# HorizonRobotics/GeoFlowSlam

Hardware: AMD Instinct MI355X
Metric: front-end frames/sec (ORB+match+GICP) on 640x480 RGBD (higher is better)
Workload: dtype u8/int32 (ORB, match) + f64 (GICP); 1 GPU; BASELINE.json configs[1]: 640x480 RGBD frame pair, ORB extract (1000 feats, 8 levels) + BF Hamming match + GMS filter + GICP on ~19k-pt clouds (stride-4 depth grid); batch_pairs_per_gpu=512, lanes_per_gpu=4, passes=K passes per lane chain, joined once, distinct_scenes_per_gpu=512, scene_seeds=1000..1511 (rank 0), global_batch_pairs=512, parallelism=frames sharded x1, no collective

## Files before the change

### geoflowslam_amd/csrc/match.hip

```cpp
#include "gfs_common.hpp"

namespace {

constexpr int kQPerBlock = 64;
constexpr int kTile = 256;

__global__ __launch_bounds__(256) void k_bf_hamming(const uint8_t* __restrict__ query, const int* __restrict__ nq_arr,
                                                    const uint8_t* __restrict__ train, const int* __restrict__ nt_arr,
                                                    int stride_rows, int* __restrict__ out_idx,
                                                    int* __restrict__ out_dist) {
  __shared__ uint4 tile[kTile * 2];
  __shared__ unsigned int part[4][kQPerBlock];
  const int b = blockIdx.y;
  const int nq = nq_arr[b], nt = nt_arr[b];
  const int q0 = blockIdx.x * kQPerBlock;
  if (q0 >= nq) return;
  const int lane = threadIdx.x & 63, wave = threadIdx.x >> 6;
  const int q = q0 + lane;
  const uint8_t* qb = query + (size_t)b * stride_rows * 32;
  const uint8_t* tb = train + (size_t)b * stride_rows * 32;

  unsigned long long qa[4] = {0, 0, 0, 0};
  if (q < nq) {
    const uint4* qp = reinterpret_cast<const uint4*>(qb + (size_t)q * 32);
    uint4 lo = qp[0], hi = qp[1];
    qa[0] = (unsigned long long)lo.x | ((unsigned long long)lo.y << 32);
    qa[1] = (unsigned long long)lo.z | ((unsigned long long)lo.w << 32);
    qa[2] = (unsigned long long)hi.x | ((unsigned long long)hi.y << 32);
    qa[3] = (unsigned long long)hi.z | ((unsigned long long)hi.w << 32);
  }
  int best = 0x7fffffff, best_j = -1;
  for (int t0 = 0; t0 < nt; t0 += kTile) {
    __syncthreads();
    const uint4* src = reinterpret_cast<const uint4*>(tb + (size_t)t0 * 32);
    const int rows = min(kTile, nt - t0);
    for (int i = threadIdx.x; i < rows * 2; i += 256) tile[i] = src[i];
    __syncthreads();
    const int r0 = wave * 64, r1 = min(r0 + 64, rows);
    for (int r = r0; r < r1; ++r) {
      uint4 lo = tile[2 * r], hi = tile[2 * r + 1];
      unsigned long long t0w = (unsigned long long)lo.x | ((unsigned long long)lo.y << 32);
      unsigned long long t1w = (unsigned long long)lo.z | ((unsigned long long)lo.w << 32);
      unsigned long long t2w = (unsigned long long)hi.x | ((unsigned long long)hi.y << 32);
      unsigned long long t3w = (unsigned long long)hi.z | ((unsigned long long)hi.w << 32);
      int d = __popcll(qa[0] ^ t0w) + __popcll(qa[1] ^ t1w) + __popcll(qa[2] ^ t2w) + __popcll(qa[3] ^ t3w);
      if (d < best) {
        best = d;
        best_j = t0 + r;
      }
    }
  }
  part[wave][lane] = best_j < 0 ? 0xffffffffu : ((unsigned int)best << 20) | (unsigned int)best_j;
  __syncthreads();
  if (wave == 0 && q < nq) {
    unsigned int k = min(min(part[0][lane], part[1][lane]), min(part[2][lane], part[3][lane]));
    int* oi = out_idx + (size_t)b * stride_rows;
    int* od = out_dist + (size_t)b * stride_rows;
    if (k == 0xffffffffu) {
      oi[q] = -1;
      od[q] = 0x7fffffff;
    } else {
      oi[q] = (int)(k & 0xfffffu);
      od[q] = (int)(k >> 20);
    }
  }
}

}

struct gfs_matcher {
  int device, max_q, max_t, max_b;
  hipStream_t stream;
  gfs::DevBuf<uint8_t> d_q, d_t;
  gfs::DevBuf<int> d_nq, d_nt, d_idx, d_dist;
  std::mutex mu;
};

extern "C" {

int gfs_hamming256(const uint8_t* a, const uint8_t* b) {
  int d = 0;
  for (int i = 0; i < 4; i++) {
    uint64_t x, y;
    memcpy(&x, a + 8 * i, 8);
    memcpy(&y, b + 8 * i, 8);
    d += __builtin_popcountll(x ^ y);
  }
  return d;
}

int gfs_matcher_create(int device, int max_query, int max_train, int max_batch, gfs_matcher** out) {
  GFS_REQUIRE(out && max_query > 0 && max_train > 0 && max_batch > 0, GFS_ERR_INVALID_ARG,
              "gfs_matcher_create: invalid argument");
  GFS_REQUIRE(max_train < (1 << 20), GFS_ERR_UNSUPPORTED, "gfs_matcher_create: max_train must be < 2^20");
  if (!gfs::device_ok(device)) return GFS_ERR_NO_DEVICE;
  GFS_HIP(hipSetDevice(device));
  gfs_matcher* h = new gfs_matcher;
  h->device = device;
  h->max_q = max_query;
  h->max_t = max_train;
  h->max_b = max_batch;
  int rc;
  GFS_HIP(hipStreamCreateWithFlags(&h->stream, hipStreamNonBlocking));
  const size_t rows = (size_t)std::max(max_query, max_train);
  if ((rc = h->d_q.alloc(rows * 32)) || (rc = h->d_t.alloc(rows * 32)) || (rc = h->d_nq.alloc(1)) ||
      (rc = h->d_nt.alloc(1)) || (rc = h->d_idx.alloc(rows)) || (rc = h->d_dist.alloc(rows))) {
    delete h;
    return rc;
  }
  *out = h;
  return GFS_OK;
}

void gfs_matcher_destroy(gfs_matcher* h) {
  if (!h) return;
  (void)hipSetDevice(h->device);
  (void)hipStreamDestroy(h->stream);
  delete h;
}

int gfs_bf_match_hamming_batch_device(gfs_matcher* h, const void* dev_query, const void* dev_nq, const void* dev_train,
                                      const void* dev_nt, int B, int stride_rows, void* dev_train_idx, void* dev_dist,
                                      void* stream) {
  GFS_REQUIRE(h && dev_query && dev_nq && dev_train && dev_nt && dev_train_idx && dev_dist && B > 0 && stride_rows > 0,
              GFS_ERR_INVALID_ARG, "gfs_bf_match_hamming_batch_device: invalid argument");
  GFS_REQUIRE(stride_rows < (1 << 20), GFS_ERR_UNSUPPORTED, "stride_rows must be < 2^20");
  GFS_HIP(hipSetDevice(h->device));
  hipStream_t s = stream ? (hipStream_t)stream : h->stream;
  dim3 grid(gfs::div_up(stride_rows, kQPerBlock), B);
  GFS_LAUNCH("k_bf_hamming", k_bf_hamming, grid, dim3(256), 0, s, (const uint8_t*)dev_query, (const int*)dev_nq,
             (const uint8_t*)dev_train, (const int*)dev_nt, stride_rows, (int*)dev_train_idx, (int*)dev_dist);
  return GFS_OK;
}

int gfs_bf_match_hamming(gfs_matcher* h, const uint8_t* query, int nq, const uint8_t* train, int nt,
                         int32_t* train_idx, int32_t* dist) {
  GFS_REQUIRE(h && nq >= 0 && nt >= 0, GFS_ERR_INVALID_ARG, "gfs_bf_match_hamming: invalid argument");
  if (nq == 0 || nt == 0) return 0;
  GFS_REQUIRE(query && train && train_idx && dist, GFS_ERR_INVALID_ARG, "gfs_bf_match_hamming: NULL buffer");
  GFS_REQUIRE(nq <= h->max_q && nt <= h->max_t, GFS_ERR_CAPACITY, "gfs_bf_match_hamming: %d x %d exceeds handle capacity %d x %d",
              nq, nt, h->max_q, h->max_t);
  std::lock_guard<std::mutex> lk(h->mu);
  GFS_HIP(hipSetDevice(h->device));
  hipStream_t s = h->stream;
  const int stride_rows = std::max(h->max_q, h->max_t);
  GFS_HIP(hipMemcpyAsync(h->d_q.p, query, (size_t)nq * 32, hipMemcpyHostToDevice, s));
  GFS_HIP(hipMemcpyAsync(h->d_t.p, train, (size_t)nt * 32, hipMemcpyHostToDevice, s));
  GFS_HIP(hipMemcpyAsync(h->d_nq.p, &nq, sizeof(int), hipMemcpyHostToDevice, s));
  GFS_HIP(hipMemcpyAsync(h->d_nt.p, &nt, sizeof(int), hipMemcpyHostToDevice, s));
  int rc = gfs_bf_match_hamming_batch_device(h, h->d_q.p, h->d_nq.p, h->d_t.p, h->d_nt.p, 1, stride_rows, h->d_idx.p,
                                             h->d_dist.p, s);
  if (rc) return rc;
  GFS_HIP(hipMemcpyAsync(train_idx, h->d_idx.p, (size_t)nq * sizeof(int), hipMemcpyDeviceToHost, s));
  GFS_HIP(hipMemcpyAsync(dist, h->d_dist.p, (size_t)nq * sizeof(int), hipMemcpyDeviceToHost, s));
  GFS_HIP(hipStreamSynchronize(s));
  return nq;
}

}
```

Baseline: 46110 frames/s.

## Compute Hamming distances with i8 MFMA over unpacked bit vectors

Replaces the popcount-based brute-force Hamming matcher with a matrix-core formulation. Train descriptor bits are unpacked to 0/1 bytes in shared memory and query bits to ±1 bytes in registers, so an int8 32x32x32 MFMA yields popcount(t) minus overlap terms, from which Hamming distance is recovered using the query popcount. Each wave handles 64 queries, the next train tile is prefetched into registers, and an argmin is kept through packed max-keys. This trades an 8x expansion in shared memory and unpack ALU work for dense matrix throughput, and the kernel now compiles only for gfx950.

```diff
diff --git a/geoflowslam_amd/csrc/match.hip b/geoflowslam_amd/csrc/match.hip
--- a/geoflowslam_amd/csrc/match.hip
+++ b/geoflowslam_amd/csrc/match.hip
@@ -1,67 +1,158 @@
 #include "gfs_common.hpp"
 
+#if defined(__HIP_DEVICE_COMPILE__) && !defined(__gfx950__)
+#error "k_bf_hamming uses v_mfma_i32_32x32x32_i8, the double-K i8 MFMA of gfx950"
+#endif
+
 namespace {
 
-constexpr int kQPerBlock = 64;
-constexpr int kTile = 256;
-
-__global__ __launch_bounds__(256) void k_bf_hamming(const uint8_t* __restrict__ query, const int* __restrict__ nq_arr,
+typedef int v4i __attribute__((ext_vector_type(4)));
+typedef int v16i __attribute__((ext_vector_type(16)));
+
+constexpr int kQB = 2;
+constexpr int kQPerBlock = 4 * 32 * kQB;
+constexpr int kTile = 128;
+constexpr int kRowStride = 256 + 16;
+
+__device__ __forceinline__ unsigned int spread4(unsigned int x) { return __umul24(x, 0x204081u) & 0x01010101u; }
+
+__device__ __forceinline__ v4i unpack01(unsigned int h) {
+  v4i r;
+  r.x = (int)spread4(h & 15u);
+  r.y = (int)spread4((h >> 4) & 15u);
+  r.z = (int)spread4((h >> 8) & 15u);
+  r.w = (int)spread4((h >> 12) & 15u);
+  return r;
+}
+
+__device__ __forceinline__ v4i unpack_pm1(unsigned int h) {
+  v4i m = unpack01(h), r;
+  r.x = (int)(0xFFFFFFFFu - (unsigned int)m.x * 0xFEu);
+  r.y = (int)(0xFFFFFFFFu - (unsigned int)m.y * 0xFEu);
+  r.z = (int)(0xFFFFFFFFu - (unsigned int)m.z * 0xFEu);
+  r.w = (int)(0xFFFFFFFFu - (unsigned int)m.w * 0xFEu);
+  return r;
+}
+
+struct KeyConsts {
+  unsigned int c[16];
+  __device__ __forceinline__ KeyConsts() {
+#pragma unroll
+    for (int r = 0; r < 16; ++r) {
+      c[r] = (256u << 20) + 32u - (unsigned int)((r & 3) + 8 * (r >> 2));
+      asm volatile("" : "+s"(c[r]));
+    }
+  }
+};
+
+template <bool kMasked>
+__device__ __forceinline__ unsigned int block_best(const v16i& acc, const KeyConsts& kc, int h4, int lim) {
+  unsigned int m = 0;
+#pragma unroll
+  for (int r = 0; r < 16; ++r) {
+    unsigned int k = ((unsigned int)acc[r] << 20) + kc.c[r];
+    if (kMasked) k = ((r & 3) + 8 * (r >> 2) + h4 < lim) ? k : 0u;
+    m = max(m, k);
+  }
+  return m;
+}
+
+__global__ __launch_bounds__(256) __attribute__((amdgpu_waves_per_eu(3))) void k_bf_hamming(const uint8_t* __restrict__ query, const int* __restrict__ nq_arr,
                                                     const uint8_t* __restrict__ train, const int* __restrict__ nt_arr,
                                                     int stride_rows, int* __restrict__ out_idx,
                                                     int* __restrict__ out_dist) {
-  __shared__ uint4 tile[kTile * 2];
-  __shared__ unsigned int part[4][kQPerBlock];
+  __shared__ __attribute__((aligned(16))) unsigned char tile[kTile * kRowStride];
   const int b = blockIdx.y;
   const int nq = nq_arr[b], nt = nt_arr[b];
   const int q0 = blockIdx.x * kQPerBlock;
   if (q0 >= nq) return;
-  const int lane = threadIdx.x & 63, wave = threadIdx.x >> 6;
-  const int q = q0 + lane;
-  const uint8_t* qb = query + (size_t)b * stride_rows * 32;
-  const uint8_t* tb = train + (size_t)b * stride_rows * 32;
-
-  unsigned long long qa[4] = {0, 0, 0, 0};
-  if (q < nq) {
-    const uint4* qp = reinterpret_cast<const uint4*>(qb + (size_t)q * 32);
-    uint4 lo = qp[0], hi = qp[1];
-    qa[0] = (unsigned long long)lo.x | ((unsigned long long)lo.y << 32);
-    qa[1] = (unsigned long long)lo.z | ((unsigned long long)lo.w << 32);
-    qa[2] = (unsigned long long)hi.x | ((unsigned long long)hi.y << 32);
-    qa[3] = (unsigned long long)hi.z | ((unsigned long long)hi.w << 32);
-  }
-  int best = 0x7fffffff, best_j = -1;
+  const int tid = threadIdx.x, lane = tid & 63, wave = tid >> 6;
+  const int col = lane & 31, h = lane >> 5;
+  const uint4* qb = reinterpret_cast<const uint4*>(query + (size_t)b * stride_rows * 32);
+  const uint4* tb = reinterpret_cast<const uint4*>(train + (size_t)b * stride_rows * 32);
+  const int wq0 = q0 + wave * (32 * kQB);
+
+  v4i bq[kQB][8];
+  int pq[kQB];
+#pragma unroll
+  for (int j = 0; j < kQB; ++j) {
+    const int q = wq0 + 32 * j + col;
+    uint4 lo = make_uint4(0, 0, 0, 0), hi = lo;
+    if (q < nq) {
+      lo = qb[2 * (size_t)q];
+      hi = qb[2 * (size_t)q + 1];
+    }
+    const unsigned int w[8] = {lo.x, lo.y, lo.z, lo.w, hi.x, hi.y, hi.z, hi.w};
+    pq[j] = 0;
+#pragma unroll
+    for (int s = 0; s < 8; ++s) {
+      pq[j] += __popc(w[s]);
+      bq[j][s] = unpack_pm1(h ? w[s] >> 16 : w[s] & 0xFFFFu);
+    }
+  }
+  unsigned int best[kQB];
+#pragma unroll
+  for (int j = 0; j < kQB; ++j) best[j] = 0u;
+
+  const int srow = tid & 127, shalf = tid >> 7;
+  unsigned char* sdst = tile + srow * kRowStride + shalf * 128;
+  const unsigned char* aread = tile + col * kRowStride + h * 16;
+  const KeyConsts kc;
+  uint4 nxt = make_uint4(0, 0, 0, 0);
+  if (srow < nt) nxt = tb[2 * (size_t)srow + shalf];
   for (int t0 = 0; t0 < nt; t0 += kTile) {
     __syncthreads();
-    const uint4* src = reinterpret_cast<const uint4*>(tb + (size_t)t0 * 32);
+    const unsigned int sw[4] = {nxt.x, nxt.y, nxt.z, nxt.w};
+#pragma unroll
+    for (int i = 0; i < 4; ++i) {
+      *reinterpret_cast<v4i*>(sdst + 32 * i) = unpack01(sw[i] & 0xFFFFu);
+      *reinterpret_cast<v4i*>(sdst + 32 * i + 16) = unpack01(sw[i] >> 16);
+    }
+    nxt = make_uint4(0, 0, 0, 0);
+    if (t0 + kTile + srow < nt) nxt = tb[2 * (size_t)(t0 + kTile + srow) + shalf];
+    __syncthreads();
+    if (wq0 >= nq) continue;
     const int rows = min(kTile, nt - t0);
-    for (int i = threadIdx.x; i < rows * 2; i += 256) tile[i] = src[i];
-    __syncthreads();
-    const int r0 = wave * 64, r1 = min(r0 + 64, rows);
-    for (int r = r0; r < r1; ++r) {
-      uint4 lo = tile[2 * r], hi = tile[2 * r + 1];
-      unsigned long long t0w = (unsigned long long)lo.x | ((unsigned long long)lo.y << 32);
-      unsigned long long t1w = (unsigned long long)lo.z | ((unsigned long long)lo.w << 32);
-      unsigned long long t2w = (unsigned long long)hi.x | ((unsigned long long)hi.y << 32);
-      unsigned long long t3w = (unsigned long long)hi.z | ((unsigned long long)hi.w << 32);
-      int d = __popcll(qa[0] ^ t0w) + __popcll(qa[1] ^ t1w) + __popcll(qa[2] ^ t2w) + __popcll(qa[3] ^ t3w);
-      if (d < best) {
-        best = d;
-        best_j = t0 + r;
+    for (int r0 = 0; r0 < rows; r0 += 32) {
+      v16i acc[kQB];
+#pragma unroll
+      for (int j = 0; j < kQB; ++j)
+#pragma unroll
+        for (int r = 0; r < 16; ++r) acc[j][r] = 0;
+#pragma unroll
+      for (int s = 0; s < 8; ++s) {
+        const v4i a = *reinterpret_cast<const v4i*>(aread + r0 * kRowStride + s * 32);
+#pragma unroll
+        for (int j = 0; j < kQB; ++j) acc[j] = __builtin_amdgcn_mfma_i32_32x32x32_i8(a, bq[j][s], acc[j], 0, 0, 0);
       }
-    }
-  }
-  part[wave][lane] = best_j < 0 ? 0xffffffffu : ((unsigned int)best << 20) | (unsigned int)best_j;
-  __syncthreads();
-  if (wave == 0 && q < nq) {
-    unsigned int k = min(min(part[0][lane], part[1][lane]), min(part[2][lane], part[3][lane]));
-    int* oi = out_idx + (size_t)b * stride_rows;
-    int* od = out_dist + (size_t)b * stride_rows;
-    if (k == 0xffffffffu) {
-      oi[q] = -1;
-      od[q] = 0x7fffffff;
-    } else {
-      oi[q] = (int)(k & 0xfffffu);
-      od[q] = (int)(k >> 20);
+      const unsigned int bc = 0xFFFFFu - 32u - (unsigned int)(t0 + r0) - 4u * (unsigned int)h;
+      if (rows - r0 >= 32) {
+#pragma unroll
+        for (int j = 0; j < kQB; ++j) best[j] = max(best[j], block_best<false>(acc[j], kc, 4 * h, 32) + bc);
+      } else {
+#pragma unroll
+        for (int j = 0; j < kQB; ++j) {
+          const unsigned int m = block_best<true>(acc[j], kc, 4 * h, rows - r0);
+          best[j] = max(best[j], m ? m + bc : 0u);
+        }
+      }
+    }
+  }
+  if (wq0 >= nq) return;
+  int* oi = out_idx + (size_t)b * stride_rows;
+  int* od = out_dist + (size_t)b * stride_rows;
+#pragma unroll
+  for (int j = 0; j < kQB; ++j) {
+    const unsigned int k = max(best[j], (unsigned int)__shfl_xor((int)best[j], 32));
+    const int q = wq0 + 32 * j + col;
+    if (h == 0 && q < nq) {
+      if (k == 0u) {
+        oi[q] = -1;
+        od[q] = 0x7fffffff;
+      } else {
+        oi[q] = (int)(0xFFFFFu - (k & 0xFFFFFu));
+        od[q] = pq[j] - ((int)(k >> 20) - 256);
+      }
     }
   }
 }
```

After: 46920 frames/s (median of 6 runs). +1.8%, better.
